# Nishad-Sharma/gpuRaytracer

Measured on AMD Instinct MI355X. Metric: Msamples/sec (pixels×spp) Cornell box 1080p at 1/2/4/8 MI355X; HBM GB/s, higher is better.
Workload: dtype f32

## Files before the change

gpuraytracer_amd/_native.py:

```python
from __future__ import annotations

import ctypes
import os

ABI_VERSION = 8
_HERE = os.path.dirname(os.path.abspath(__file__))
library_path = os.environ.get("RTPT_LIB") or os.path.join(_HERE, "librtpt.so")


class float3(ctypes.Structure):

    _fields_ = [("x", ctypes.c_float), ("y", ctypes.c_float), ("z", ctypes.c_float),
                ("_pad", ctypes.c_float)]

    def __iter__(self):
        return iter((self.x, self.y, self.z))


class float4(ctypes.Structure):
    _fields_ = [("x", ctypes.c_float), ("y", ctypes.c_float), ("z", ctypes.c_float),
                ("w", ctypes.c_float)]


class int2(ctypes.Structure):
    _fields_ = [("x", ctypes.c_int32), ("y", ctypes.c_int32)]


class MaterialGPU(ctypes.Structure):
    _fields_ = [("diffuse", float4), ("metallic", ctypes.c_float),
                ("roughness", ctypes.c_float), ("_pad", ctypes.c_float * 2),
                ("emissive", float3)]


class SphereGPU(ctypes.Structure):
    _fields_ = [("center", float3), ("material", MaterialGPU), ("radius", ctypes.c_float),
                ("_pad", ctypes.c_float * 3)]


# ... 115 lines not shown
    "rt_place_tiles_host": (ctypes.c_int, [_P, ctypes.c_int32, ctypes.c_int32, ctypes.c_int32,
                                           ctypes.c_uint32, _P]),
    "rt_build_sha": (ctypes.c_char_p, []),
    "rt_debug_stats": (ctypes.c_int, [_P, _P, ctypes.c_int]),
    "rt_last_error": (ctypes.c_char_p, [_P]),
    "rt_status_string": (ctypes.c_char_p, [ctypes.c_int]),
    "rt_abi_version": (ctypes.c_int, []),
    "rt_seed_splitmix": (None, [ctypes.c_uint64, _P, ctypes.c_size_t]),
    "rt_scene_cornell_box": (ctypes.c_int, [ctypes.c_int32, ctypes.c_int32,
                                            ctypes.POINTER(CameraGPU),
                                            ctypes.POINTER(MaterialGPU),
                                            ctypes.POINTER(float3),
                                            ctypes.POINTER(SquareLightGPU),
                                            ctypes.POINTER(ctypes.c_uint32)]),
    "rt_scene_random_spheres": (ctypes.c_int, [ctypes.c_int32, ctypes.c_int32, ctypes.c_uint32,
                                               ctypes.c_uint64, ctypes.POINTER(CameraGPU),
                                               ctypes.POINTER(MaterialGPU),
                                               ctypes.POINTER(float3),
                                               ctypes.POINTER(SquareLightGPU),
                                               ctypes.POINTER(ctypes.c_uint32),
                                               ctypes.POINTER(SphereGPU)]),
    "rt_render_mis": (ctypes.c_int, [_P, ctypes.POINTER(MisParamsC), _P, _P]),
    "rt_scene_cornell_box_mis": (ctypes.c_int, [ctypes.c_int32, ctypes.c_int32,
                                                ctypes.POINTER(CameraGPU),
                                                ctypes.POINTER(MaterialGPU),
                                                ctypes.POINTER(float3),
                                                ctypes.POINTER(SquareLightGPU),
                                                ctypes.POINTER(ctypes.c_uint32)]),
    "rt_tonemap_rgba8": (None, [_P, ctypes.c_size_t, _P]),
    "rt_scene_describe": (ctypes.c_int, [ctypes.POINTER(SceneDesc), ctypes.POINTER(SceneInfo)]),
    "rt_scene_describe_ex": (ctypes.c_int, [ctypes.POINTER(SceneDesc), ctypes.POINTER(CreateOptions),
                                            ctypes.POINTER(SceneInfo)]),
    "rt_debug_camera_candidates": (ctypes.c_int, [ctypes.POINTER(SceneDesc)] + [ctypes.c_int32] * 4 + [_P]),
}


class RtError(RuntimeError):

    def __init__(self, status: int, message: str):
        super().__init__(f"{STATUS.get(status, status)}: {message}")
        self.status = status


def _preload_hip_runtime():
    if os.environ.get("RTPT_SYSTEM_HIP") == "1":
        return
    import importlib.util
    spec = importlib.util.find_spec("torch")
    if spec is None or not spec.submodule_search_locations:
        return
    for d in spec.submodule_search_locations:
        cand = os.path.join(d, "lib", "libamdhip64.so")
        if os.path.exists(cand):
            ctypes.CDLL(cand, mode=ctypes.RTLD_GLOBAL)
            return


def _load():
    if not os.path.exists(library_path):
        raise ImportError(
            f"{library_path} is missing: build the HIP extension first "
            "(`make` or `python -c 'import __graft_entry__ as g; g.build()'`). "
            "There is no CPU fallback.")
    _preload_hip_runtime()
    handle = ctypes.CDLL(library_path)
    for name, (res, args) in SIGNATURES.items():
# ... 21 lines not shown
```

gpuraytracer_amd/csrc/rt_api.cpp:

```cpp
#include <hip/hip_runtime.h>
#include <rccl/rccl.h>

#include <stdio.h>
#include <stdlib.h>
#include <string.h>

#include <algorithm>
#include <chrono>
#include <new>
#include <string>
#include <vector>

#include "../../include/rtpt.h"
#include "rt_beam.hpp"
#include "rt_kernel.hpp"
#include "rt_scene.hpp"

constexpr uint32_t kDefaultTriBuild = RT_TRI_BVH_GPU_SAH;

struct rt_ctx {
    int device = 0;
    hipStream_t stream = nullptr;
    rt::CompiledScene scene;
    float4* d_tri_isect = nullptr;
    float4* d_tri_shade = nullptr;
    float4* d_pair_isect = nullptr;
    float4* d_clusters = nullptr;
    uint32_t* d_sph_lds = nullptr;
    uint16_t* d_sph_lds_id = nullptr;
    uint4* d_sph_box = nullptr;
    float4* d_sph_isect = nullptr;
    float4* d_sph_shade = nullptr;
    float4* d_sph_nodes = nullptr;
    uint32_t* d_sph_perm = nullptr;
    uint4* d_tri_nodes = nullptr;
    uint32_t tri_build = kDefaultTriBuild;
    float4* d_tri_sorted = nullptr;
    uint32_t* d_tri_perm = nullptr;
    uint32_t tri_bvh_nodes = 0;
    uint32_t tri_bvh_build_used = 0;
    float tri_bvh_build_ms = 0.0f;
    size_t tri_bvh_temp_bytes = 0;
    float scene_compile_ms = 0.0f;
    float4* d_mis_shade = nullptr;
    float4* d_mis_tab = nullptr;
    uint32_t mis_tab_S = 0;
    void* d_out8 = nullptr;
// ... 958 lines not shown
    const size_t lds_clu =
        lds + (info->n_spheres ? 0u : rt::kCluF4 * sizeof(float) * 4 * info->n_box_clusters);
    info->lds_bytes = (!bvh && lds <= rt::kMaxLdsBytes)
                          ? (uint32_t)(lds_clu <= rt::kMaxLdsBytes ? lds_clu : lds)
                          : 0u;
    const rt::KernelChoice kc =
        rt::choose_kernel(info->n_triangles, info->n_triangle_pairs, info->n_spheres, info->n_box_clusters,
                          info->n_triangle_bvh_nodes, rt::sphere_compact_usable(s), 3, ro.mem, ro.walk);
    info->kernel_layout = (uint32_t)kc.layout;
    info->kernel_lds_bytes = (uint32_t)kc.lds_bytes;
    return RT_OK;
}

int rt_debug_camera_candidates(const rt_scene_desc* d, int32_t x0, int32_t x1, int32_t y0, int32_t y1,
                               uint8_t* may_hit) {
    if (!d || !may_hit || !d->camera || !d->square_lights || x1 < x0 || y1 < y0 || x0 < 0 || y0 < 0)
        return fail(nullptr, RT_ERR_INVALID_ARG, "null argument or empty rectangle");
    rt::CompiledScene s;
    const char* err = nullptr;
    if (!rt::compile_scene(*d->camera, d->materials, d->vertices, d->n_triangles, d->square_lights[0],
                           d->spheres, d->n_spheres, &s, &err))
        return fail(nullptr, RT_ERR_INVALID_ARG, err);
    memset(may_hit, 1, d->n_triangles);
    const rt::CamConst& c = s.cam;
    const rt::Beam beam = rt::make_beam(rt::f3{c.pos[0], c.pos[1], c.pos[2]}, rt::f3{c.u[0], c.u[1], c.u[2]},
                                        rt::f3{c.v[0], c.v[1], c.v[2]}, rt::f3{c.w[0], c.w[1], c.w[2]}, c.halfW,
                                        c.halfH, (float)c.W, (float)c.H, (float)(uint32_t)x0, (float)(uint32_t)x1,
                                        (float)(uint32_t)y0, (float)(uint32_t)y1);
    for (size_t k = 0; k < s.pair_isect.size(); ++k)
        if (rt::beam_excludes_pair(beam, s.pair_isect[k].q)) may_hit[2 * k] = may_hit[2 * k + 1] = 0;
    return RT_OK;
}

int rt_debug_stats(rt_ctx* c, uint64_t* out, int n) {
    if (!c || !out || n <= 0) return fail(c, RT_ERR_INVALID_ARG, "null argument");
    DeviceGuard g(c->device);
    hipError_t e = rt::read_debug_stats(reinterpret_cast<unsigned long long*>(out), n);
    if (e == hipErrorNotSupported) return fail(c, RT_ERR_STATE, "not an RT_STATS build");
    if (e != hipSuccess) return hip_fail(c, RT_ERR_LAUNCH, "read stats", e);
    return RT_OK;
}

void rt_seed_splitmix(uint64_t key, uint32_t* seeds, size_t n) {
    if (!seeds) return;
    for (size_t p = 0; p < n; ++p) seeds[p] = rt::seed_splitmix(key, p);
}

static void fill_scene_arrays(const rt::Scene& s, CameraGPU* camera, MaterialGPU* materials,
                              rt_float3* vertices, SquareLightGPU* light) {
    *camera = rt::convert_camera(s.camera);
    for (size_t k = 0; k < s.triangles.size(); ++k) {
        materials[k] = rt::convert_material(s.triangles[k].material);
        for (int v = 0; v < 3; ++v) vertices[3 * k + v] = rt::to_abi(s.triangles[k].vertices[v]);
    }
    *light = rt::convert_square_light(s.light);
}

int rt_scene_cornell_box(int32_t width, int32_t height, CameraGPU* camera, MaterialGPU* materials,
                         rt_float3* vertices, SquareLightGPU* light, uint32_t* n_triangles) {
    if (!camera || !materials || !vertices || !light || !n_triangles || width <= 0 || height <= 0)
        return RT_ERR_INVALID_ARG;
    const rt::Scene s = rt::init_cornell_box(width, height);
    fill_scene_arrays(s, camera, materials, vertices, light);
    *n_triangles = (uint32_t)s.triangles.size();
    return RT_OK;
}
// ... 32 lines not shown
```

gpuraytracer_amd/csrc/rt_kernel.hip:

```cpp
#include <hip/hip_runtime.h>
#include <hip/hip_fp16.h>

#include <stddef.h>
#include <stdio.h>
#ifdef RT_LDS_CHECK
#include <hsa/hsa.h>
#endif

#include "rt_kernel.hpp"
#include "rt_halton.hpp"
#include "rt_beam.hpp"
#include "rt_trace.hpp"

namespace rt {

#ifdef RT_LDS_CHECK
__device__ uint32_t g_lds_overflow;
__device__ __forceinline__ bool lds_short(size_t end) {
    const uint32_t grp = ((const uint32_t*)__builtin_amdgcn_dispatch_ptr())[7];
    const size_t dyn = grp - __builtin_amdgcn_groupstaticsize();
    if (end <= dyn) return false;
    if (threadIdx.x == 0) atomicMax(&g_lds_overflow, (uint32_t)end);
    return true;
}
static_assert(offsetof(hsa_kernel_dispatch_packet_t, group_segment_size) == 28, "AQL packet layout");
#define RT_LDS_GUARD(end)            \
    do {                             \
        if (lds_short(end)) return;  \
    } while (0)
#else
#define RT_LDS_GUARD(end) ((void)0)
#endif

namespace {

#ifndef RT_CENSUS
#define RT_CENSUS 0
#endif
#ifndef RT_LQ
#define RT_LQ 1
#endif
template <typename T>
__device__ __forceinline__ T cz(T v) {
    asm volatile("" : "+v"(v));
// ... 490 lines not shown
    const uint32_t kWX = (L == 1) ? 8u : P.wave_w, kWY = (64u / L) / kWX;
    uint32_t bx, by;
    {
        constexpr uint32_t kXcdRun = 4;
        const uint32_t n = gridDim.x * gridDim.y, full = n / (8u * kXcdRun + (kXcdRun == 0)) * (8u * kXcdRun);
        const uint32_t p = blockIdx.y * gridDim.x + blockIdx.x;
        uint32_t t = p;
        if (kXcdRun > 0 && p < full) {
            const uint32_t xcd = p % 8u, k = p / 8u;
            t = ((k / kXcdRun) * 8u + xcd) * kXcdRun + k % kXcdRun;
        }
        bx = t % gridDim.x;
        by = t / gridDim.x;
    }
    auto pixel_of = [&](uint32_t t, uint32_t& x, uint32_t& j) {
        const uint32_t lane = t & 63u, wave = t >> 6, pix = lane / L;
        x = bx * (WR * kWX) + (wave % WR) * kWX + (pix % kWX);
        j = by * (WC * kWY) + (wave / WR) * kWY + (pix / kWX);
    };
    if constexpr (RT_CAM_CAND && GEO == kGeoPairClu) {
        if (sv.nP - 1u < 32u) {
            const uint32_t wave = wave_uniform(threadIdx.x >> 6);
            const uint32_t wx0 = bx * (WR * kWX) + (wave % WR) * kWX;
            const uint32_t wj0 = by * (WC * kWY) + (wave / WR) * kWY;
            const float y0 = (float)(P.row_start + wj0 * P.row_step);
            const float y1 = (float)(P.row_start + (wj0 + kWY - 1u) * P.row_step);
            const Beam beam = make_beam(ld_f3(P.cam_pos), ld_f3(P.cam_u), ld_f3(P.cam_v), ld_f3(P.cam_w), P.halfW,
                                        P.halfH, (float)P.W, (float)P.H, (float)wx0, (float)(wx0 + kWX - 1u), y0, y1);
            const uint32_t k = threadIdx.x & 63u;
            const uint32_t kc = min(k, sv.nP - 1u);
            const bool keep = !beam_excludes_pair(beam, reinterpret_cast<const float*>(sv.pair + kPairF4 * kc));
            sv.cam_mask = wave_uniform((uint32_t)__builtin_amdgcn_ballot_w64(k < sv.nP && keep));
            sv.cam_avail = true;
        }
    }
    constexpr bool kRemat = GEO == kGeoPairClu || GEO == kGeoSphLds;
    auto opaque_tid = []() {
        uint32_t t = threadIdx.x;
        if constexpr (kRemat) asm volatile("" : "+v"(t));
        return t;
    };
    {
        uint32_t x, j;
        pixel_of(threadIdx.x, x, j);
        if (x >= (uint32_t)P.W || j >= P.row_count) return;
    }
    __shared__ uint32_t seed_s[NT];
    __shared__ float lum_s[L > 1 ? 3 * (NT / L) : 1];
    f3 lum{0.0f, 0.0f, 0.0f};
    {
        const uint32_t t = threadIdx.x, sub = t % L;
        uint32_t x, j;
        pixel_of(t, x, j);
        const uint32_t y = P.row_start + j * P.row_step;
        seed_s[t] = P.seeds[(size_t)y * (size_t)P.W + x] + P.sample_base;
        if (P.accumulate) {
            const float4 prev = P.sum[(size_t)j * (size_t)P.W + x];
            lum = f3{prev.x, prev.y, prev.z};
        }
        const uint32_t slot = t / L;
        if (L > 1 && sub == 0) {
            lum_s[3 * slot] = lum.x;
            lum_s[3 * slot + 1] = lum.y;
            lum_s[3 * slot + 2] = lum.z;
        }
    }
// ... 538 lines not shown
```

gpuraytracer_amd/csrc/rt_kernel.hpp:

```cpp
#pragma once

#include <hip/hip_runtime.h>
#include <stddef.h>
#include <stdint.h>

#include "rt_math.h"

namespace rt {

constexpr uint32_t kBlockThreads = 256;
constexpr uint32_t kTile = 16;
constexpr size_t kMaxLdsBytes = 64 * 1024;
constexpr uint32_t kOutFp16 = 0x2u;
constexpr uint32_t kOutRgba8 = 0x10u;
constexpr uint32_t kPairF4 = 7;
constexpr uint32_t kSphBlockThreads = 64;
constexpr size_t kSphPairLdsMaxBytes = 6 * 1024;
constexpr uint32_t kCluF4 = 7;
#ifndef RT_CAM_CAND
#define RT_CAM_CAND 1
#endif
constexpr uint32_t kTriCompactLayouts = 8;
constexpr uint32_t kTriBvhMinTriangles = 384;

struct KParams {
    const float4* tri_isect;
    const float4* pair_isect;
    const float4* tri_shade;
    const float4* sph_isect;
    const float4* sph_nodes;
    const uint32_t* sph_perm;
    const float4* sph_shade;
    const uint32_t* sph_lds;
    const uint16_t* sph_lds_id;
    const uint4* sph_box;
    const uint4* tri_nodes;
    const float4* tri_sorted;
    const uint32_t* tri_perm;
    const uint32_t* seeds;
    float4* sum;
    void* out;
    uint32_t nT, nP, nS, nN;
    uint32_t nE;
    uint32_t nTN;
    float cam_pos[3], cam_u[3], cam_v[3], cam_w[3];
    float halfW, halfH;
    int32_t W, H;
    float light_center[3], light_color[3];
    uint32_t spp, sample_base;
    uint32_t row_start, row_step, row_count;
    uint32_t accumulate;
    uint32_t samples_total;
    uint32_t flags;
// ... 98 lines not shown
```

gpuraytracer_amd/csrc/rt_trace.hpp:

```cpp
#pragma once
#include <hip/hip_runtime.h>

#include "rt_kernel.hpp"

namespace rt {
namespace {

__device__ __forceinline__ f3 ld_f3(const float* p) { return f3{p[0], p[1], p[2]}; }

__device__ __forceinline__ bool tri_test(const float4& A, const float4& Bq, const float4& C, f3 o,
                                         f3 d, float tmin, float tmax, float* t_out) {
    const f3 v0{A.x, A.y, A.z}, e1{A.w, Bq.x, Bq.y}, e2{Bq.z, Bq.w, C.x}, n{C.y, C.z, C.w};
    const f3 tv = o - v0;
    const f3 c = cross(tv, d);
    const float den = dot(n, d);
    const uint32_t sgn = __float_as_uint(den) & 0x80000000u;
    const uint32_t nsgn = sgn ^ 0x80000000u;
    const float bu = __uint_as_float(__float_as_uint(dot(e2, c)) ^ nsgn);
    const float bv = __uint_as_float(__float_as_uint(dot(e1, c)) ^ sgn);
    const float aden = fabsf(den);
    if (aden > 0.0f && bu >= 0.0f && bv >= 0.0f && bu + bv <= aden) {
        const float tn = __uint_as_float(__float_as_uint(dot(n, tv)) ^ nsgn);
        const float t = tn / aden;
        if (t > tmin && t < tmax) {
// ... 72 lines not shown
#define RT_STAT(slot, v) stat_wave((slot), (v))
#else
#define RT_STAT(slot, v) ((void)0)
#endif

enum Geo : int {
    kGeoTriLds = 0,
    kGeoPairLds = 1,
    kGeoPairSmem = 4,
    kGeoTriBvh = 5,
    kGeoTriGlobal = 2,
    kGeoPairClu = 6,
    kGeoSphLds = 7,
};

constexpr bool geo_pairs(int g) { return g == kGeoPairLds || g == kGeoPairSmem || g == kGeoSphLds; }

struct SceneView {
    const float4* tri;
    const float4* pair;
    const float4* sph;
    const float4* node;
    const uint32_t* sph_perm;
    const uint4* tnode;
    const float4* tsorted;
    const uint32_t* tperm;
    uint32_t nTN;
    uint32_t nT, nP, nS, nN;
    const float4* clu;
    uint32_t nC;
    uint32_t pair_free;
    uint32_t cam_mask = 0;
    bool cam_avail = false;
    const float* htab;
    const uint4* sent;
    const uint16_t* sid;
    const uint4* sbox;
    uint32_t nSB;
    const float4* shade;
    float* xstash;
};

__device__ __forceinline__ float vmin(float a, float b) {
    float r;
    asm("v_min_f32 %0, %1, %2" : "=v"(r) : "v"(a), "v"(b));
    return r;
}
__device__ __forceinline__ float vmax(float a, float b) {
    float r;
    asm("v_max_f32 %0, %1, %2" : "=v"(r) : "v"(a), "v"(b));
    return r;
}
__device__ __forceinline__ float vmin3(float a, float b, float c) {
    float r;
    asm("v_min3_f32 %0, %1, %2, %3" : "=v"(r) : "v"(a), "v"(b), "v"(c));
    return r;
}
__device__ __forceinline__ float vmax3(float a, float b, float c) {
    float r;
    asm("v_max3_f32 %0, %1, %2, %3" : "=v"(r) : "v"(a), "v"(b), "v"(c));
    return r;
}

struct RayBox {
    f3 invd, oinv;
};
// ... 465 lines not shown
            for (int q = 1; q < RT_TRI_CHK; ++q) {
                RT_STAT(ST + 2, 1);
                RT_STAT(ST + 3, __popcll(__builtin_amdgcn_ballot_w64(idx < end && leaf == kNone)));
                if (idx < end && leaf == kNone) {
                    const uint4 e = cn[idx];
                    const bool inner = (e.w & 0x80000000u) != 0u;
                    const bool h = lds_node_hit_nf(e, rb, tmin, best);
                    leaf = (h && !inner) ? e.w : leaf;
                    idx = (h || !inner) ? idx + 1 : (e.w & 0x7FFFFFFFu);
                }
            }
#endif
            const int parked = __popcll(__builtin_amdgcn_ballot_w64(leaf != kNone));
            const int live = __popcll(__builtin_amdgcn_ballot_w64(idx < end || leaf != kNone));
            if (kTriParkDen * parked >= live) break;
        }
        if (__builtin_amdgcn_ballot_w64(leaf != kNone) == 0) break;
        RT_STAT(ST + 5, 1);
        RT_STAT(ST + 6, __popcll(__builtin_amdgcn_ballot_w64(leaf != kNone)));
        if (leaf != kNone) {
            if (ANY) {
                if (tri_leaf_any(tri, leaf, o, d, tmin, best)) {
                    id = 0;
                    idx = end;
                }
            } else {
                tri_leaf_closest(tri, perm, leaf, o, d, tmin, best, id);
            }
            leaf = kNone;
        }
    }
}

template <bool SEG = false>
__device__ __forceinline__ uint32_t cluster_candidates(const SceneView& sv, f3 o, f3 d, float tmin,
                                                       float tmax) {
    constexpr float kEps = 1.52587890625e-05f;
    uint32_t skip = 0;
    if (SEG) {
        const f3 e = o + d * tmax;
        for (uint32_t c = 0; c < sv.nC; ++c) {
            const float4* r = sv.clu + kCluF4 * c;
            if (!(__float_as_uint(r[3].w) & 8u)) continue;
            const float4 X = r[0], Y = r[1], Z = r[2];
            const bool inside = o.x > X.x && o.x < X.y && e.x > X.x && e.x < X.y &&
                                o.y > Y.x && o.y < Y.y && e.y > Y.x && e.y < Y.y &&
                                o.z > Z.x && o.z < Z.y && e.z > Z.x && e.z < Z.y;
            if (__builtin_amdgcn_ballot_w64(!inside) == 0) skip |= 1u << c;
        }
    }
    const RayBox rb = ray_box(o, d);
    const float iv[3] = {rb.invd.x, rb.invd.y, rb.invd.z};
    const float oi[3] = {rb.oinv.x, rb.oinv.y, rb.oinv.z};
    uint32_t mask = 0;
    uint32_t c = 0;
    for (; c < sv.nC; ++c) {
        if (SEG && ((skip >> c) & 1u)) continue;
        const float4* r = sv.clu + kCluF4 * c;
        const float4 H = r[3], W = r[6];
        const float4 M0 = r[4], M1 = r[5];
        const uint32_t flags = __float_as_uint(H.w);
        if (flags & 16u) break;
        const float hi[3] = {H.x, H.y, H.z}, wf[3] = {W.x, W.y, W.z};
        float en[3], ex[3], ida[3];
#pragma unroll
        for (int a = 0; a < 3; ++a) {
            const float4 A = r[a];
            float t0, t1;
            if (flags & (1u << a)) {
                ida[a] = iv[a];
                t0 = fmaf(A.w, iv[a], -oi[a]);
                t1 = fmaf(hi[a], iv[a], -oi[a]);
            } else {
                const float oa = dot(f3{A.x, A.y, A.z}, o), da = dot(f3{A.x, A.y, A.z}, d);
                ida[a] = safe_rcp(da);
                t0 = (A.w - oa) * ida[a];
                t1 = (hi[a] - oa) * ida[a];
            }
            en[a] = vmin(t0, t1);
            ex[a] = vmax(t0, t1);
        }
        const float tlo0 = vmax3(en[0], en[1], vmax(en[2], tmin));
        const float thi0 = vmin3(ex[0], ex[1], vmin(ex[2], tmax));
        const float tlo = fmaf(-kEps, fabsf(tlo0), tlo0), thi = fmaf(kEps, fabsf(thi0), thi0);
        if (!__builtin_amdgcn_ballot_w64(tlo <= thi)) continue;
        const uint32_t m[6] = {__float_as_uint(M0.x), __float_as_uint(M0.y), __float_as_uint(M0.z),
                               __float_as_uint(M0.w), __float_as_uint(M1.x), __float_as_uint(M1.y)};
        uint32_t cm = 0;
#pragma unroll
        for (int a = 0; a < 3; ++a) {
            const bool neg = ida[a] < 0.0f;
            const uint32_t m_en = neg ? m[2 * a + 1] : m[2 * a];
            const uint32_t m_ex = neg ? m[2 * a] : m[2 * a + 1];
            const float wa = wf[a] * fabsf(ida[a]);
            cm |= (en[a] + fmaf(fabsf(en[a]), kEps, wa) >= tlo) ? m_en : 0u;
            cm |= (ex[a] - fmaf(fabsf(ex[a]), kEps, wa) <= thi) ? m_ex : 0u;
        }
        mask |= (tlo <= thi) ? cm : 0u;
    }
    for (; c < sv.nC; ++c) {
        const float4* r = sv.clu + kCluF4 * c;
        const float4 A0 = r[0], A1 = r[1], A2 = r[2], H = r[3];
        const uint32_t flags = __float_as_uint(H.w);
        const float4 A[3] = {A0, A1, A2};
        const float hi[3] = {H.x, H.y, H.z};
        float tlo0 = tmin, thi0 = tmax;
#pragma unroll
        for (int a = 0; a < 3; ++a) {
            float t0, t1;
            if (flags & (1u << a)) {
                t0 = fmaf(A[a].w, iv[a], -oi[a]);
                t1 = fmaf(hi[a], iv[a], -oi[a]);
            } else {
                const float oa = dot(f3{A[a].x, A[a].y, A[a].z}, o);
                const float ida = safe_rcp(dot(f3{A[a].x, A[a].y, A[a].z}, d));
                t0 = (A[a].w - oa) * ida;
                t1 = (hi[a] - oa) * ida;
            }
            tlo0 = vmax(tlo0, vmin(t0, t1));
            thi0 = vmin(thi0, vmax(t0, t1));
        }
        const float tlo = fmaf(-kEps, fabsf(tlo0), tlo0), thi = fmaf(kEps, fabsf(thi0), thi0);
        mask |= (tlo <= thi) ? __float_as_uint(r[5].z) : 0u;
    }
    return mask;
}

#ifndef RT_PAIR_SEL
#define RT_PAIR_SEL 0
#endif
template <bool ANY>
__device__ __forceinline__ void pair_test_rank(const float4* r, uint32_t k, f3 o, f3 d, float tmin,
                                               float* best, int* id) {
// ... 27 lines not shown
            const int ib = (int)(2 * k + 1);
            if (t2 > tmin && (t2 < *best || (!ANY && t2 == *best && ib < *id))) {
                if (!ANY) *best = t2;
                *id = ib;
            }
        }
    }
}

#ifndef RT_CLU_HELP
#define RT_CLU_HELP 0
#endif
__device__ __forceinline__ uint32_t select_bit64(uint64_t m, uint32_t r) {
    uint32_t pos = 0;
    uint32_t lo = (uint32_t)m;
    uint32_t c = (uint32_t)__builtin_popcount(lo);
    if (r >= c) {
        r -= c;
        pos = 32;
        lo = (uint32_t)(m >> 32);
    }
#pragma unroll
    for (uint32_t w = 16; w >= 1; w >>= 1) {
        c = (uint32_t)__builtin_popcount(lo & ((1u << w) - 1u));
        if (r >= c) {
            r -= c;
            pos += w;
            lo >>= w;
        }
    }
    return pos;
}

template <bool ANY, bool SEG = ANY>
__device__ __forceinline__ void cluster_query(const SceneView& sv, f3 o, f3 d, float tmin,
                                              float* best, int* id) {
    for (uint32_t free = sv.pair_free; free != 0u; free &= free - 1u) {
        const uint32_t k = (uint32_t)__builtin_ctz(free);
        pair_test_rank<ANY>(sv.pair + kPairF4 * k, k, o, d, tmin, best, id);
    }
    uint32_t cand = cluster_candidates<SEG>(sv, o, d, tmin, *best);
    RT_STAT(12, 1);
    RT_STAT(15, __popcll(__ballot(1)));
#if RT_CLU_HELP
    const uint32_t me = __lane_id();
    for (;;) {
        const bool want = cand != 0u && !(ANY && *id >= 0);
        if (__builtin_amdgcn_ballot_w64(want) == 0) break;
        const bool two = want && (cand & (cand - 1u)) != 0u;
        const uint64_t m2 = __builtin_amdgcn_ballot_w64(two);
        const uint64_t idle = __builtin_amdgcn_ballot_w64(!want);
        const uint32_t n2 = (uint32_t)__popcll(m2), ni = (uint32_t)__popcll(idle);
        uint32_t partner = me;
        bool helped = false, helping = false;
        if (two) {
            const uint32_t q = (uint32_t)__popcll(m2 & ((1ull << me) - 1ull));
            if (q < ni) {
                partner = select_bit64(idle, q);
                helped = true;
            }
        } else if (!want) {
            const uint32_t r = (uint32_t)__popcll(idle & ((1ull << me) - 1ull));
            if (r < n2) {
                partner = select_bit64(m2, r);
                helping = true;
            }
        }
        const f3 po{__shfl(o.x, (int)partner), __shfl(o.y, (int)partner), __shfl(o.z, (int)partner)};
        const f3 pd{__shfl(d.x, (int)partner), __shfl(d.y, (int)partner), __shfl(d.z, (int)partner)};
        const uint32_t pc = (uint32_t)__shfl((int)cand, (int)partner);
        const float ob = __shfl(*best, (int)partner);
        const int oid = __shfl(*id, (int)partner);
        float tb = helping ? ob : *best;
        int tid = helping ? oid : *id;
// ... 94 lines not shown
    } else if (GEO == kGeoTriBvh) {
        if (CULL)
            tri_cbvh_closest_packet(sv.tnode, sv.tsorted, sv.tperm, sv.nTN, o, d, tmin,
                                    best, id);
        else
            tri_cbvh_walk<false>(sv.tnode, sv.tsorted, sv.tperm, sv.nTN, o, d, tmin,
                                 best, id);
    } else {
        for (uint32_t k = 0; k < sv.nT; ++k) {
            float t;
            if (tri_test(sv.tri[3 * k], sv.tri[3 * k + 1], sv.tri[3 * k + 2], o, d, tmin, best,
                         &t)) {
                best = t;
                id = (int)k;
            }
        }
    }
    if (SPH && GEO == kGeoSphLds && RT_SPH_LEAFBOX)
        sphere_walk_box<false>(sv.sbox, sv.sph, sv.sph_perm, sv.nSB, sv.nT, o, d, tmin, best, id);
    else if (SPH && GEO == kGeoSphLds)
        sphere_walk<false>(sv.sent, sv.sid, sv.nN, sv.nT, o, d, tmin, best, id);
    else if (SPH)
        sphere_closest(sv.node, sv.sph, sv.sph_perm, sv.nN, sv.nT, o, d, tmin, best, id);
    *t_io = best;
    return id;
}

template <int GEO, bool SPH, bool PACKET>
__device__ __forceinline__ bool any_hit(const SceneView& sv, f3& o, f3& d, float tmin, float tmax,
                                        f3 seg_lo, f3 seg_hi) {
    if (GEO == kGeoPairClu) {
        float tm = tmax;
        int id = -1;
        cluster_query<true>(sv, o, d, tmin, &tm, &id);
        if (id >= 0) return true;
    } else if (geo_pairs(GEO)) {
        for (uint32_t k = 0; k < sv.nP; ++k) {
            const float4* r = sv.pair + kPairF4 * k;
            const float4 b0 = r[5], b1 = r[6];
            const bool overlap = seg_lo.x <= b0.w && seg_hi.x >= b0.x && seg_lo.y <= b1.x &&
                                 seg_hi.y >= b0.y && seg_lo.z <= b1.y && seg_hi.z >= b0.z;
            RT_STAT(8, 1);
            if (!__any(overlap)) continue;
            RT_STAT(9, 1);
            RT_STAT(10, __popcll(__ballot(1)));
            const float4 r0 = r[0], r1 = r[1], r2 = r[2], r3 = r[3], r4 = r[4];
            const PairDots q = pair_dots(r0, r1, r2, r3, r4, o, d);
            const bool pa = bary_ok(q.denA, q.a1, q.a2);
            const bool pb = bary_ok(q.denB, q.b1, q.b2);
            if (pa || pb) {
                RT_STAT(11, 1);
                const f3 nsel = pa ? f3{r2.y, r2.z, r2.w} : f3{r3.w, r4.x, r4.y};
                const float t = pair_t(nsel, q.tv, pa ? q.denA : q.denB);
                if (t > tmin && t < tmax) return true;
                if (pa && pb) {
                    const float t2 = pair_t(f3{r3.w, r4.x, r4.y}, q.tv, q.denB);
                    if (t2 > tmin && t2 < tmax) return true;
                }
            }
        }
    } else if (GEO == kGeoTriBvh) {
        if (PACKET) {
            if (tri_cbvh_any_packet(sv.tnode, sv.tsorted, sv.nTN, o, d, tmin, tmax))
                return true;
        } else {
            float tm = tmax;
            int hid = -1;
// ... 140 lines not shown
```

include/rtpt.h:

```cpp
#ifndef RTPT_H
#define RTPT_H

#include "rt_types.h"

#ifdef __cplusplus
extern "C" {
#endif

#define RTPT_ABI_VERSION 8

#define RT_MAX_BOUNCES 4

typedef enum rt_status {
    RT_OK = 0,
    RT_ERR_INVALID_ARG = 1,
    RT_ERR_NO_DEVICE = 2,
    RT_ERR_OUT_OF_MEMORY = 3,
    RT_ERR_LAUNCH = 4,
    RT_ERR_STATE = 5,
    RT_ERR_COMM = 6
} rt_status;

typedef struct rt_ctx rt_ctx;

typedef struct rt_scene_desc {
    const CameraGPU* camera;
    const MaterialGPU* materials;
    const SquareLightGPU* square_lights;
    uint32_t n_square_lights;
    const rt_float3* vertices;
    uint32_t n_triangles;
    const SphereGPU* spheres;
    uint32_t n_spheres;
    int32_t device;
} rt_scene_desc;

#define RT_OUT_DEVICE 0x1u
#define RT_OUT_FP16   0x2u
#define RT_OUT_NONE   0x4u
#define RT_KEEP_SUM   0x8u
#define RT_OUT_RGBA8  0x10u

// ... 136 lines not shown
typedef struct rt_mis_params {
    uint32_t camera_rays;
    uint32_t mis_samples;
    uint32_t row_start, row_step, row_count;
    uint32_t flags;
} rt_mis_params;

int rt_render_mis(rt_ctx* ctx, const rt_mis_params* params, float* out_rgba32f,
                  uint8_t* out_rgba8);

int rt_scene_cornell_box_mis(int32_t width, int32_t height, CameraGPU* camera,
                             MaterialGPU* materials, rt_float3* vertices,
                             SquareLightGPU* light, uint32_t* n_triangles);

typedef struct rt_scene_info {
    uint32_t n_triangles;
    uint32_t n_triangle_pairs;
    uint32_t n_spheres;
    uint32_t lds_bytes;
    uint32_t n_sphere_nodes;
    uint32_t n_triangle_bvh_nodes;
    uint32_t n_box_clusters;
    uint32_t pair_free_mask;
    uint32_t sphere_kernel_lds_bytes;
    uint32_t kernel_layout;
    uint32_t kernel_lds_bytes;
} rt_scene_info;
int rt_scene_describe(const rt_scene_desc* scene, rt_scene_info* info);
int rt_scene_describe_ex(const rt_scene_desc* scene, const rt_create_options* opt, rt_scene_info* info);

int rt_debug_camera_candidates(const rt_scene_desc* scene, int32_t x0, int32_t x1, int32_t y0, int32_t y1,
                               uint8_t* may_hit);

void rt_tonemap_rgba8(const float* rgba32f, size_t n_pixels, uint8_t* rgba8);

#ifdef __cplusplus
}
#endif

#endif
```

Before: 24550.

## Cull shadow-ray occluder candidates per wave using camera-beam-to-light shaft tests

Adds conservative shaft culling. When a wave's camera beam hits exactly one triangle pair, the code builds a shaft from that pair's beam footprint to the square light and tests every pair and cluster against it. The resulting masks restrict which pairs and clusters shadow (any-hit) rays test, and the shadow ray returns immediately when nothing can occlude. This adds per-wave setup math and extra branches, and correctness depends on the conservative epsilon bounds.

```diff
diff --git a/gpuraytracer_amd/_native.py b/gpuraytracer_amd/_native.py
--- a/gpuraytracer_amd/_native.py
+++ b/gpuraytracer_amd/_native.py
@@ -3,7 +3,7 @@
 import ctypes
 import os
 
-ABI_VERSION = 8
+ABI_VERSION = 9
 _HERE = os.path.dirname(os.path.abspath(__file__))
 library_path = os.environ.get("RTPT_LIB") or os.path.join(_HERE, "librtpt.so")
 
@@ -185,6 +185,8 @@
     "rt_scene_describe_ex": (ctypes.c_int, [ctypes.POINTER(SceneDesc), ctypes.POINTER(CreateOptions),
                                             ctypes.POINTER(SceneInfo)]),
     "rt_debug_camera_candidates": (ctypes.c_int, [ctypes.POINTER(SceneDesc)] + [ctypes.c_int32] * 4 + [_P]),
+    "rt_debug_shadow_candidates": (ctypes.c_int, [ctypes.POINTER(SceneDesc)] + [ctypes.c_int32] * 4 +
+                                   [_P, ctypes.POINTER(ctypes.c_int32)]),
 }
 
 
diff --git a/gpuraytracer_amd/csrc/rt_api.cpp b/gpuraytracer_amd/csrc/rt_api.cpp
--- a/gpuraytracer_amd/csrc/rt_api.cpp
+++ b/gpuraytracer_amd/csrc/rt_api.cpp
@@ -13,6 +13,7 @@
 
 #include "../../include/rtpt.h"
 #include "rt_beam.hpp"
+#include "rt_shaft.hpp"
 #include "rt_kernel.hpp"
 #include "rt_scene.hpp"
 
@@ -1037,6 +1038,45 @@
     return RT_OK;
 }
 
+int rt_debug_shadow_candidates(const rt_scene_desc* d, int32_t x0, int32_t x1, int32_t y0, int32_t y1,
+                               uint8_t* may_occlude, int32_t* available) {
+    if (!d || !may_occlude || !available || !d->camera || !d->square_lights || x1 < x0 || y1 < y0 || x0 < 0 ||
+        y0 < 0)
+        return fail(nullptr, RT_ERR_INVALID_ARG, "null argument or empty rectangle");
+    rt::CompiledScene s;
+    const char* err = nullptr;
+    if (!rt::compile_scene(*d->camera, d->materials, d->vertices, d->n_triangles, d->square_lights[0],
+                           d->spheres, d->n_spheres, &s, &err))
+        return fail(nullptr, RT_ERR_INVALID_ARG, err);
+    memset(may_occlude, 1, d->n_triangles);
+    *available = 0;
+    const size_t nP = s.pair_isect.size();
+    if (nP == 0) return RT_OK;
+    const rt::CamConst& c = s.cam;
+    const rt::Beam beam = rt::make_beam(rt::f3{c.pos[0], c.pos[1], c.pos[2]}, rt::f3{c.u[0], c.u[1], c.u[2]},
+                                        rt::f3{c.v[0], c.v[1], c.v[2]}, rt::f3{c.w[0], c.w[1], c.w[2]}, c.halfW,
+                                        c.halfH, (float)c.W, (float)c.H, (float)(uint32_t)x0, (float)(uint32_t)x1,
+                                        (float)(uint32_t)y0, (float)(uint32_t)y1);
+    const rt::ShaftLight L = rt::shaft_light(rt::f3{s.light.center[0], s.light.center[1], s.light.center[2]});
+    std::vector<uint8_t> keep(nP, 0);
+    bool ok = true;
+    for (size_t k = 0; k < nP; ++k) {
+        if (rt::beam_excludes_pair(beam, s.pair_isect[k].q)) continue;
+        for (int tb = 0; tb < 2; ++tb) {
+            const float* sh = s.tri_shade[2 * k + tb].s;
+            if (sh[3] != 0.0f) continue;
+            const rt::ShaftSrc S = rt::shaft_source(beam, s.pair_isect[k].q, tb, rt::f3{sh[0], sh[1], sh[2]}, L);
+            ok = ok && S.ok;
+            for (size_t j = 0; j < nP; ++j)
+                if (!rt::shaft_excludes_pair(S, L, s.pair_isect[j].q)) keep[j] = 1;
+        }
+    }
+    if (!ok) return RT_OK;
+    *available = 1;
+    for (size_t j = 0; j < nP; ++j) may_occlude[2 * j] = may_occlude[2 * j + 1] = keep[j];
+    return RT_OK;
+}
+
 int rt_debug_stats(rt_ctx* c, uint64_t* out, int n) {
     if (!c || !out || n <= 0) return fail(c, RT_ERR_INVALID_ARG, "null argument");
     DeviceGuard g(c->device);
diff --git a/gpuraytracer_amd/csrc/rt_kernel.hip b/gpuraytracer_amd/csrc/rt_kernel.hip
--- a/gpuraytracer_amd/csrc/rt_kernel.hip
+++ b/gpuraytracer_amd/csrc/rt_kernel.hip
@@ -10,6 +10,7 @@
 #include "rt_kernel.hpp"
 #include "rt_halton.hpp"
 #include "rt_beam.hpp"
+#include "rt_shaft.hpp"
 #include "rt_trace.hpp"
 
 namespace rt {
@@ -566,6 +567,30 @@
             const bool keep = !beam_excludes_pair(beam, reinterpret_cast<const float*>(sv.pair + kPairF4 * kc));
             sv.cam_mask = wave_uniform((uint32_t)__builtin_amdgcn_ballot_w64(k < sv.nP && keep));
             sv.cam_avail = true;
+            if constexpr (RT_SHD_CAND) {
+                const uint32_t tb = k >> 5, kt = min(k & 31u, sv.nP - 1u);
+                bool occ = false, bad = (sv.cam_mask & (sv.cam_mask - 1u)) != 0u;
+                if (sv.cam_mask != 0u && !bad) {
+                    const uint32_t sp = (uint32_t)__builtin_ctz(sv.cam_mask);
+                    const float4 s0 = P.tri_shade[4 * (2u * sp + tb)];
+                    if (s0.w == 0.0f) {
+                        const ShaftLight lq = shaft_light(ld_f3(P.light_center));
+                        const ShaftSrc src = shaft_source(beam, reinterpret_cast<const float*>(sv.pair + kPairF4 * sp),
+                                                          (int)tb, f3{s0.x, s0.y, s0.z}, lq);
+                        bad = !src.ok;
+                        occ = !shaft_excludes_pair(src, lq, reinterpret_cast<const float*>(sv.pair + kPairF4 * kt));
+                    }
+                }
+                const unsigned long long ob = __builtin_amdgcn_ballot_w64((k & 31u) < sv.nP && occ);
+                sv.shd_mask = wave_uniform((uint32_t)ob | (uint32_t)(ob >> 32));
+                sv.shd_avail = __builtin_amdgcn_ballot_w64(bad) == 0ull && sv.nC <= 32u;
+                if (sv.nC != 0u) {
+                    const uint32_t kc2 = min(k, sv.nC - 1u);
+                    const uint32_t all = __float_as_uint(reinterpret_cast<const float*>(sv.clu + kCluF4 * kc2)[22]);
+                    sv.shd_cskip = wave_uniform(
+                        (uint32_t)__builtin_amdgcn_ballot_w64(k < sv.nC && (all & sv.shd_mask) == 0u));
+                }
+            }
         }
     }
     constexpr bool kRemat = GEO == kGeoPairClu || GEO == kGeoSphLds;
diff --git a/gpuraytracer_amd/csrc/rt_kernel.hpp b/gpuraytracer_amd/csrc/rt_kernel.hpp
--- a/gpuraytracer_amd/csrc/rt_kernel.hpp
+++ b/gpuraytracer_amd/csrc/rt_kernel.hpp
@@ -19,6 +19,9 @@
 constexpr uint32_t kCluF4 = 7;
 #ifndef RT_CAM_CAND
 #define RT_CAM_CAND 1
+#endif
+#ifndef RT_SHD_CAND
+#define RT_SHD_CAND 1
 #endif
 constexpr uint32_t kTriCompactLayouts = 8;
 constexpr uint32_t kTriBvhMinTriangles = 384;
diff --git a/gpuraytracer_amd/csrc/rt_shaft.hpp b/gpuraytracer_amd/csrc/rt_shaft.hpp
--- /dev/null
+++ b/gpuraytracer_amd/csrc/rt_shaft.hpp
@@ -0,0 +1,185 @@
+#pragma once
+
+#include "rt_beam.hpp"
+
+namespace rt {
+
+#ifndef RT_SHAFT_FAM
+#define RT_SHAFT_FAM 15
+#endif
+
+constexpr float kShaftEps = 3.814697265625e-06f;
+constexpr float kShaftBig = 1e15f;
+
+struct ShaftLight {
+    f3 q[4];
+    float qmax;
+    bool ok;
+};
+
+RT_HD ShaftLight shaft_light(f3 c) {
+    ShaftLight L;
+    L.ok = true;
+    L.qmax = 0.0f;
+    for (int i = 0; i < 4; ++i) {
+        const float ux = (i == 1 || i == 2) ? 1.0f : -1.0f, uy = i >= 2 ? 1.0f : -1.0f;
+        const f3 a{c.x + 0.25f * ux, c.y, c.z + 0.25f * uy};
+        const f3 b = (c + f3{0.25f, 0.0f, 0.0f} * ux) + f3{0.0f, 0.0f, 0.25f} * uy;
+        L.q[i] = a;
+        const float l = sqrtf(dot(a, a));
+        L.ok = L.ok && a.x == b.x && a.y == b.y && a.z == b.z && l < kShaftBig;
+        L.qmax = fmaxf(L.qmax, l);
+    }
+    return L;
+}
+
+RT_HD float shaft_pair_pad(const float* q, f3 w[4]) {
+    const f3 v0{q[0], q[1], q[2]}, S{q[3], q[4], q[5]}, eA{q[6], q[7], q[8]}, eB{q[12], q[13], q[14]};
+    const f3 lo{q[20], q[21], q[22]}, hi{q[23], q[24], q[25]};
+    w[0] = v0;
+    w[1] = v0 + S;
+    w[2] = v0 + eA;
+    w[3] = v0 + eB;
+    f3 mn = w[0], mx = w[0];
+    for (int j = 1; j < 4; ++j) {
+        mn = f3{fminf(mn.x, w[j].x), fminf(mn.y, w[j].y), fminf(mn.z, w[j].z)};
+        mx = f3{fmaxf(mx.x, w[j].x), fmaxf(mx.y, w[j].y), fmaxf(mx.z, w[j].z)};
+    }
+    return fmaxf(fmaxf(fmaxf(mn.x - lo.x, mn.y - lo.y), mn.z - lo.z),
+                 fmaxf(fmaxf(hi.x - mx.x, hi.y - mx.y), hi.z - mx.z));
+}
+
+struct ShaftSrc {
+    f3 p[4];
+    f3 pc;
+    float rho;
+    float smax;
+    float xmax;
+    float dmax;
+    bool ok;
+};
+
+RT_HD ShaftSrc shaft_source(const Beam& B, const float* rec, int tb, f3 N, const ShaftLight& L) {
+    ShaftSrc S;
+    const f3 v0{rec[0], rec[1], rec[2]};
+    const f3 n = tb ? f3{rec[15], rec[16], rec[17]} : f3{rec[9], rec[10], rec[11]};
+    const float nl = sqrtf(dot(n, n));
+    const float num = dot(n, v0 - B.apex);
+    const float al = sqrtf(dot(B.apex, B.apex)), vl = sqrtf(dot(v0, v0));
+    bool ok = B.ok && L.ok && nl > 0.0f && nl < kShaftBig && al < kShaftBig && vl < kShaftBig;
+    const float den0 = dot(n, B.b[0]);
+    float cmin = 1e30f, pmax = 0.0f;
+    f3 sum{0.0f, 0.0f, 0.0f};
+    for (int i = 0; i < 4; ++i) {
+        const float den = dot(n, B.b[i]);
+        const float t = num / den;
+        ok = ok && fabsf(den) > kBeamEps * (nl * B.bl[i]) && (den > 0.0f) == (den0 > 0.0f) && t > 0.0f && t < kShaftBig;
+        S.p[i] = (B.apex + B.b[i] * t) + N * 1e-3f;
+        sum = sum + S.p[i];
+        cmin = fminf(cmin, fabsf(den) / (nl * B.bl[i]));
+        const float pl = sqrtf(dot(S.p[i], S.p[i]));
+        ok = ok && pl < kShaftBig;
+        pmax = fmaxf(pmax, pl);
+    }
+    S.pc = sum * 0.25f;
+    float dq = 0.0f, dp = 0.0f;
+    for (int j = 0; j < 4; ++j) {
+        const f3 a = L.q[j] - S.p[0], b = S.p[j] - S.p[0];
+        dq = fmaxf(dq, sqrtf(dot(a, a)));
+        dp = fmaxf(dp, sqrtf(dot(b, b)));
+    }
+    const float dmax = (dq + dp) * 1.001f;
+    S.dmax = dmax;
+    S.smax = 1.0f - 1e-3f / dmax;
+    ok = ok && dmax > 2e-3f && S.smax > 0.0f && S.smax < 1.0f;
+    S.xmax = fmaxf(pmax, L.qmax);
+    const float scale = (al + vl) + 2.0f * (pmax + L.qmax);
+    S.rho = kShaftEps * (scale / cmin);
+    ok = ok && S.rho >= 0.0f && S.rho < 1e30f;
+    S.ok = ok;
+    return S;
+}
+
+RT_HD void shaft_extents(const ShaftSrc& S, const ShaftLight& L, f3 n, float* pl, float* ph, float* ql,
+                         float* qh) {
+    *pl = *ph = dot(n, S.p[0]);
+    *ql = *qh = dot(n, L.q[0]);
+    for (int i = 1; i < 4; ++i) {
+        const float a = dot(n, S.p[i]), b = dot(n, L.q[i]);
+        *pl = fminf(*pl, a);
+        *ph = fmaxf(*ph, a);
+        *ql = fminf(*ql, b);
+        *qh = fmaxf(*qh, b);
+    }
+}
+
+RT_HD void shaft_range(const ShaftSrc& S, const ShaftLight& L, f3 n, float* lo, float* hi) {
+    float pl, ph, ql, qh;
+    shaft_extents(S, L, n, &pl, &ph, &ql, &qh);
+    *lo = fminf(pl, pl + S.smax * (ql - pl));
+    *hi = fmaxf(ph, ph + S.smax * (qh - ph));
+}
+
+RT_HD bool shaft_axis_separates(const ShaftSrc& S, const ShaftLight& L, f3 n, f3 a, f3 b, f3 c, float m,
+                                float wmax) {
+    const float nl = sqrtf(dot(n, n));
+    if (!(nl > 1e-30f && nl < kShaftBig)) return false;
+    float lo, hi;
+    shaft_range(S, L, n, &lo, &hi);
+    const float ta = dot(n, a), tb = dot(n, b), tc = dot(n, c);
+    const float tlo = fminf(fminf(ta, tb), tc), thi = fmaxf(fmaxf(ta, tb), tc);
+    const float gap = (m + kShaftEps * (S.xmax + wmax)) * nl;
+    return lo - thi > gap || tlo - hi > gap;
+}
+
+RT_HD bool shaft_ends_on_plane(const ShaftSrc& S, const ShaftLight& L, f3 n, f3 v0, float wmax) {
+    const float nl = sqrtf(dot(n, n));
+    if (!(nl > 1e-30f && nl < kShaftBig)) return false;
+    float pl, ph, ql, qh;
+    shaft_extents(S, L, n, &pl, &ph, &ql, &qh);
+    const float t0 = dot(n, v0);
+    const float eta = fmaxf(fabsf(qh - t0), fabsf(ql - t0)) / nl;
+    const float gap = fmaxf(ql - ph, pl - qh) - (S.rho + kShaftEps * S.xmax) * nl;
+    const float cosmin = gap / (nl * (S.dmax + S.rho));
+    const float tround = 1.1920929e-07f * S.dmax;
+    return tround < 0.5e-3f && eta + kShaftEps * (3.0f * S.xmax + wmax) < (0.5e-3f - tround) * cosmin;
+}
+
+RT_HD bool shaft_misses_triangle(const ShaftSrc& S, const ShaftLight& L, f3 n, f3 a, f3 b, f3 c, float ma,
+                                 float m, float wmax) {
+    if ((RT_SHAFT_FAM & 1) && shaft_axis_separates(S, L, n, a, b, c, ma, wmax)) return true;
+    if ((RT_SHAFT_FAM & 8) && shaft_ends_on_plane(S, L, n, a, wmax)) return true;
+    if (RT_SHAFT_FAM & 4) {
+        const f3 e[3] = {b - a, c - b, a - c};
+        for (int k = 0; k < 3; ++k)
+            for (int j = 0; j < 4; ++j)
+                if (shaft_axis_separates(S, L, cross(e[k], L.q[j] - S.pc), a, b, c, m, wmax)) return true;
+    }
+    return false;
+}
+
+RT_HD bool shaft_excludes_pair(const ShaftSrc& S, const ShaftLight& L, const float* q) {
+    if (!S.ok) return false;
+    f3 w[4];
+    const float pad = shaft_pair_pad(q, w);
+    if (!(pad >= 0.0f && pad < 1e30f)) return false;
+    float wmax = 0.0f;
+    for (int j = 0; j < 4; ++j) wmax = fmaxf(wmax, sqrtf(dot(w[j], w[j])));
+    if (!(wmax < kShaftBig)) return false;
+    if (RT_SHAFT_FAM & 2) {
+        const float lo[3] = {q[20], q[21], q[22]}, hi[3] = {q[23], q[24], q[25]};
+        const float gap = S.rho + kShaftEps * (S.xmax + wmax);
+        for (int a = 0; a < 3; ++a) {
+            float slo, shi;
+            shaft_range(S, L, f3{a == 0 ? 1.0f : 0.0f, a == 1 ? 1.0f : 0.0f, a == 2 ? 1.0f : 0.0f}, &slo, &shi);
+            if (slo - hi[a] > gap || lo[a] - shi > gap) return true;
+        }
+    }
+    const float m = S.rho + 2.0f * pad;
+    const float ma = S.rho + kShaftEps * (3.0f * S.xmax + wmax);
+    const f3 nA{q[9], q[10], q[11]}, nB{q[15], q[16], q[17]};
+    return shaft_misses_triangle(S, L, nA, w[0], w[1], w[2], ma, m, wmax) &&
+           shaft_misses_triangle(S, L, nB, w[0], w[1], w[3], ma, m, wmax);
+}
+
+}
diff --git a/gpuraytracer_amd/csrc/rt_trace.hpp b/gpuraytracer_amd/csrc/rt_trace.hpp
--- a/gpuraytracer_amd/csrc/rt_trace.hpp
+++ b/gpuraytracer_amd/csrc/rt_trace.hpp
@@ -128,6 +128,9 @@
     uint32_t pair_free;
     uint32_t cam_mask = 0;
     bool cam_avail = false;
+    uint32_t shd_mask = 0;
+    uint32_t shd_cskip = 0;
+    bool shd_avail = false;
     const float* htab;
     const uint4* sent;
     const uint16_t* sid;
@@ -659,14 +662,15 @@
     }
 }
 
-template <bool SEG = false>
+template <bool SEG = false, bool ALLOW = false>
 __device__ __forceinline__ uint32_t cluster_candidates(const SceneView& sv, f3 o, f3 d, float tmin,
-                                                       float tmax) {
+                                                       float tmax, uint32_t cskip = 0u) {
     constexpr float kEps = 1.52587890625e-05f;
     uint32_t skip = 0;
     if (SEG) {
         const f3 e = o + d * tmax;
         for (uint32_t c = 0; c < sv.nC; ++c) {
+            if (ALLOW && ((cskip >> c) & 1u)) continue;
             const float4* r = sv.clu + kCluF4 * c;
             if (!(__float_as_uint(r[3].w) & 8u)) continue;
             const float4 X = r[0], Y = r[1], Z = r[2];
@@ -682,8 +686,12 @@
     uint32_t mask = 0;
     uint32_t c = 0;
     for (; c < sv.nC; ++c) {
+        const float4* r = sv.clu + kCluF4 * c;
+        if (ALLOW && ((cskip >> c) & 1u)) {
+            if (__float_as_uint(r[3].w) & 16u) break;
+            continue;
+        }
         if (SEG && ((skip >> c) & 1u)) continue;
-        const float4* r = sv.clu + kCluF4 * c;
         const float4 H = r[3], W = r[6];
         const float4 M0 = r[4], M1 = r[5];
         const uint32_t flags = __float_as_uint(H.w);
@@ -726,6 +734,7 @@
         mask |= (tlo <= thi) ? cm : 0u;
     }
     for (; c < sv.nC; ++c) {
+        if (ALLOW && ((cskip >> c) & 1u)) continue;
         const float4* r = sv.clu + kCluF4 * c;
         const float4 A0 = r[0], A1 = r[1], A2 = r[2], H = r[3];
         const uint32_t flags = __float_as_uint(H.w);
@@ -819,14 +828,15 @@
     return pos;
 }
 
-template <bool ANY, bool SEG = ANY>
+template <bool ANY, bool SEG = ANY, bool ALLOW = false>
 __device__ __forceinline__ void cluster_query(const SceneView& sv, f3 o, f3 d, float tmin,
                                               float* best, int* id) {
-    for (uint32_t free = sv.pair_free; free != 0u; free &= free - 1u) {
+    for (uint32_t free = ALLOW ? (sv.pair_free & sv.shd_mask) : sv.pair_free; free != 0u; free &= free - 1u) {
         const uint32_t k = (uint32_t)__builtin_ctz(free);
         pair_test_rank<ANY>(sv.pair + kPairF4 * k, k, o, d, tmin, best, id);
     }
-    uint32_t cand = cluster_candidates<SEG>(sv, o, d, tmin, *best);
+    uint32_t cand = cluster_candidates<SEG, ALLOW>(sv, o, d, tmin, *best, ALLOW ? sv.shd_cskip : 0u);
+    if (ALLOW) cand &= sv.shd_mask;
     RT_STAT(12, 1);
     RT_STAT(15, __popcll(__ballot(1)));
 #if RT_CLU_HELP
@@ -987,7 +997,12 @@
     if (GEO == kGeoPairClu) {
         float tm = tmax;
         int id = -1;
-        cluster_query<true>(sv, o, d, tmin, &tm, &id);
+        if (RT_SHD_CAND && RT_CAM_CAND && PACKET && sv.shd_avail) {
+            if (sv.shd_mask == 0u) return false;
+            cluster_query<true, true, true>(sv, o, d, tmin, &tm, &id);
+        } else {
+            cluster_query<true>(sv, o, d, tmin, &tm, &id);
+        }
         if (id >= 0) return true;
     } else if (geo_pairs(GEO)) {
         for (uint32_t k = 0; k < sv.nP; ++k) {
diff --git a/include/rtpt.h b/include/rtpt.h
--- a/include/rtpt.h
+++ b/include/rtpt.h
@@ -7,7 +7,7 @@
 extern "C" {
 #endif
 
-#define RTPT_ABI_VERSION 8
+#define RTPT_ABI_VERSION 9
 
 #define RT_MAX_BOUNCES 4
 
@@ -210,6 +210,9 @@
 int rt_debug_camera_candidates(const rt_scene_desc* scene, int32_t x0, int32_t x1, int32_t y0, int32_t y1,
                                uint8_t* may_hit);
 
+int rt_debug_shadow_candidates(const rt_scene_desc* scene, int32_t x0, int32_t x1, int32_t y0, int32_t y1,
+                               uint8_t* may_occlude, int32_t* available);
+
 void rt_tonemap_rgba8(const float* rgba32f, size_t n_pixels, uint8_t* rgba8);
 
 #ifdef __cplusplus
```

Result: faster. 25650, median of 6 (+4.5%).
